# wzf2000/GAMER

Hardware: AMD Instinct MI355X
Metric: train-step sequences/sec, Qwen3Multi SMB decoder, his_len=100 (higher is better)
Workload: dtype f32 tensors/accumulators, products = 3 x fp16 pieces (split3)

## Files before the change

### gamer_amd/csrc/attention_common.h

```cpp
#pragma once
#include "common.h"
#include <stdlib.h>

namespace gamer {

constexpr int AT_THREADS = 256;
constexpr int KLD = 68;
constexpr int INT_BIG_A = 0x7fffffff;

typedef float f32x16 __attribute__((ext_vector_type(16)));
__device__ __forceinline__ int rowmap(int reg, int h) { return (reg & 3) + 8 * (reg >> 2) + 4 * h; }

struct RowOrder {
    const int32_t* perm;
    const int32_t* tile_kind;
    const int32_t* tile_maxpos;
    const int32_t* span;
};

struct QuerySpan {
    int hi, hole_lo, hole_hi;
    template <bool SPAN>
    static __device__ __forceinline__ QuerySpan load(const int32_t* __restrict__ span, int64_t tok, int pos, bool valid, int S) {
        QuerySpan q;
// ... 68 lines not shown
            v.x = ok ? v.x : 0.f; v.y = ok ? v.y : 0.f; v.z = ok ? v.z : 0.f; v.w = ok ? v.w : 0.f;
            *reinterpret_cast<float4*>(lds + (f >> 4) * LD + ((f & 15) << 2)) = v;
        }
    }
}

struct KeyMeta {
    int32_t kl[32];
    uint32_t kw[32];
    int32_t klmax;
    int32_t pad_[3];
};

template <bool DROP>
__device__ __forceinline__ int key_meta_load(const int32_t* __restrict__ klb, int j0, int S, int w, int lane,
                                             const AttnDropout& rng) {
    const int j = j0 + (lane & 31);
    int v = 0;
    if (w == 0 || w == 1) {
        v = j < S ? klb[j] : INT_BIG_A;
    } else if (w == 2) {
        if (DROP) v = (int)rng.key_word((uint32_t)j);
    }
    return v;
}
__device__ __forceinline__ void key_meta_store(KeyMeta& km, int w, int lane, int v) {
    if (w == 0) { if (lane < 32) km.kl[lane] = v; }
    else if (w == 1) { v = wave_max_i32(v); if (lane == 0) km.klmax = v; }
    else if (w == 2) { if (lane < 32) km.kw[lane] = (uint32_t)v; }
}

__device__ __forceinline__ void read_key_quads(const int32_t* __restrict__ base, int h, int (&out)[16]) {
#pragma unroll
    for (int g4 = 0; g4 < 4; ++g4) {
        const int4 t = *reinterpret_cast<const int4*>(base + 8 * g4 + 4 * h);
        out[4 * g4] = t.x; out[4 * g4 + 1] = t.y; out[4 * g4 + 2] = t.z; out[4 * g4 + 3] = t.w;
    }
}

constexpr float RESCALE_TAU = 20.f;

template <typename T>
struct AttnFwdArgs {
    const T* q; int ldq; const T* k; int ldk; const T* v; int ldv;
    const int32_t* kl; const int32_t* ql; const int32_t* row_empty;
    int B, S, nq, nkv; float scale, p_drop; uint64_t seed;
    T* o; float* lse;
    RowOrder ro; int uspan;
    hipStream_t st;
};
template <typename T>
struct AttnBwdArgs {
    const T* q; int ldq; const T* k; int ldk; const T* v; int ldv;
    const T* o; const T* d_o; const float* lse; float* delta;
    const int32_t* kl; const int32_t* ql; const int32_t* row_empty; const int32_t* tile_empty;
    int B, S, nq, nkv; float scale, p_drop; uint64_t seed;
    T* dq; int lddq; T* dk; int lddk; T* dv; int lddv;
    RowOrder ro; float* ds_work; int delta_ready;
    hipStream_t st;
};
template <typename F>
static inline int with_group(int nq, int nkv, F&& f) {
    return nq / nkv == 1 ? f(std::integral_constant<int, 1>{}) : f(std::integral_constant<int, 2>{});
}

static inline int check_attn(const char* name, bool bf16, const void* q, const void* k, const void* v, const void* kl,
                             const void* row_empty, int ldq, int ldk, int ldv, int B, int S, int nq, int nkv, float p_drop) {
    GAMER_CHECK_ARG(q && k && v && kl && (bf16 || row_empty), "%s: null pointer", name);
    GAMER_CHECK_ARG(B > 0 && S > 0 && nq > 0 && nkv > 0 && nq % nkv == 0, "%s: bad shape B=%d S=%d nq=%d nkv=%d", name, B, S, nq, nkv);
    const int G = nq / nkv, m = bf16 ? 8 : 4;
    GAMER_CHECK_ARG(G == 1 || G == 2, "%s: GQA group %d not built (1 or 2)", name, G);
    GAMER_CHECK_ARG(ldq % m == 0 && ldk % m == 0 && ldv % m == 0 && ldq >= nq * 64 && ldk >= nkv * 64 && ldv >= nkv * 64,
                    "%s: bad leading dims ldq=%d ldk=%d ldv=%d%s", name, ldq, ldk, ldv, bf16 ? " (multiples of 8)" : "");
    GAMER_CHECK_ARG(aligned16(q) && aligned16(k) && aligned16(v), "%s: q/k/v must be 16-byte aligned", name);
    GAMER_CHECK_ARG(p_drop >= 0.f && p_drop < 1.f, "%s: p_drop=%f", name, p_drop);
    return 0;
}

static inline bool res_enabled() {
    static EnvSwitch sw("GAMER_ATTN_RES");
    return sw.get(1) != 0;
}
#define GAMER_RES_PART(name) ([]() -> bool { static EnvSwitch sw(name); return sw.get(1) != 0; }())
static inline int res_grid_cap() {
    static EnvSwitch grid("GAMER_ATTN_RES_GRID");
    if (grid.get(0) > 0) return grid.get(0);
    static int cap[MAX_DEVICES] = {};
    int& c = cap[current_device()];
    if (c == 0) {
        int n = 0;
        if (hipDeviceGetAttribute(&n, hipDeviceAttributeMultiprocessorCount, current_device()) != hipSuccess) n = 256;
        c = n > 0 ? n : 256;
    }
    return c;
}
static inline int res_split(int n_pairs, int ways) {
    if (ways < 2) return 0;
    static EnvSwitch sp("GAMER_ATTN_RES_SPLIT");
    if (sp.is_set()) return sp.get(0) != 0;
    const int ncu = res_grid_cap();
    const double whole = (double)((n_pairs + ncu - 1) / ncu), halves = 0.58 * (double)((ways * n_pairs + ncu - 1) / ncu);
    return halves < whole ? 1 : 0;
}
static inline bool res_split_forced() { static EnvSwitch sp("GAMER_ATTN_RES_SPLIT"); return sp.is_set(); }
static inline double res_fill(int n_pairs) {
    const int ncu = res_grid_cap();
    if (n_pairs <= ncu) return 1.0;
    return (double)n_pairs / ((double)((n_pairs + ncu - 1) / ncu) * ncu);
}
static inline dim3 res_grid(int n_units) { return dim3(n_units < res_grid_cap() ? n_units : res_grid_cap()); }

}
```

### gamer_amd/csrc/attention_res.hip

```cpp
#include "attention_split_common.h"

namespace gamer {

#ifndef RES_WARM
#define RES_WARM 0
#endif
#ifndef RES_TOUCH_Q
#define RES_TOUCH_Q 0
#endif
#ifndef RES_PREFETCH_Q
#define RES_PREFETCH_Q 0
#endif
#ifndef RES_STAMP
#define RES_STAMP 0
#endif
#if RES_STAMP
__device__ unsigned long long* g_res_stamp = nullptr;
#define RES_MARK(i) do { __builtin_amdgcn_sched_barrier(0); const unsigned long long t_ = __builtin_amdgcn_s_memtime(); \
                         ph_[i] += (t_ - tprev_); tprev_ = t_; __builtin_amdgcn_sched_barrier(0); } while (0)
#define RES_STAMP_ARGS , unsigned long long (&ph_)[8], unsigned long long& tprev_
#define RES_STAMP_PASS , ph_, tprev_
#else
#define RES_MARK(i) do { } while (0)
#define RES_STAMP_ARGS
// ... 272 lines not shown
#pragma unroll
            for (int reg = 0; reg < 16; ++reg) {
                float pe = __builtin_amdgcn_exp2f(st[reg]);
                if (EMPTYSEL) pe = my_empty ? 1.f : pe;
                rowsum += pe;
                st[reg] = pe;
            }
            rowsum = xor32_sum(rowsum);
            l_run += rowsum;
            if (DROP) {
                int kwv[16];
                read_key_quads(kwt, h, kwv);
#pragma unroll
                for (int reg = 0; reg < 16; ++reg) st[reg] = rng.keep(aw, (uint32_t)kwv[reg]) ? st[reg] : 0.f;
            }
            pv_tile.template operator()<false>();
        };
        if (wave_all_empty) {
            int kwv[16];
            if (DROP) read_key_quads(kwt, h, kwv);
#pragma unroll
            for (int reg = 0; reg < 16; ++reg) {
                const bool on = DROP ? rng.keep(aw, (uint32_t)kwv[reg]) : true;
                st[reg] = on ? 1.f : 0.f;
            }
            pv_tile.template operator()<true>();
        } else if (wave_has_empty) {
            softmax_tile.template operator()<true, true>();
        } else {
            const int klmax = __builtin_amdgcn_readfirstlane(sm.klmax[tl]);
            const bool free_tile = (j0 + 31 <= wave_q_lo) && (klmax < wave_ql_min) &&
                                   (!SPAN || j0 + 31 < wave_hole_lo || j0 >= wave_hole_hi);
            if (free_tile) softmax_tile.template operator()<false, false>();
            else softmax_tile.template operator()<true, false>();
        }
#if RES_STAMP
        ph_[6] += 1;
#endif
    }
    RES_MARK(2);

    if (last) {
        float omax = 0.f;
        if (valid_q) {
            float linv = my_empty ? invS : (l_run > 0.f ? 1.f / l_run : 0.f);
            if (DROP) linv *= rng.scale;
            linv *= H2Scales::INV_P * sc.inv_v;
#pragma unroll
            for (int dh = 0; dh < 2; ++dh)
#pragma unroll
                for (int g4 = 0; g4 < 4; ++g4) {
                    float4 t4;
                    t4.x = oacc[dh][4 * g4 + 0] * linv; t4.y = oacc[dh][4 * g4 + 1] * linv;
                    t4.z = oacc[dh][4 * g4 + 2] * linv; t4.w = oacc[dh][4 * g4 + 3] * linv;
                    *reinterpret_cast<float4*>(orow + 32 * dh + 8 * g4 + 4 * h) = t4;
                    omax = fmaxf(fmaxf(fmaxf(omax, fabsf(t4.x)), fabsf(t4.y)), fmaxf(fabsf(t4.z), fabsf(t4.w)));
                }
            if (h == 0) *lse_p = my_empty ? 0.f : (m_ref + __log2f(l_run)) * 0.6931471805599453f;
        }
        if (want_amax) {
            uint32_t mw = __float_as_uint(omax);
#pragma unroll
            for (int o2 = 32; o2 > 0; o2 >>= 1) mw = max(mw, (uint32_t)__shfl_xor((int)mw, o2, 64));
            if (lane == 0 && mw) atomicMax(&sm.amax_word, mw);
        }
    } else if (valid_q) {
        float f = my_empty ? 1.f : (l_run > 0.f ? 1.f / l_run : 0.f);
        f *= H2Scales::INV_P * sc.inv_v;
#pragma unroll
        for (int dh = 0; dh < 2; ++dh)
#pragma unroll
            for (int g4 = 0; g4 < 4; ++g4) {
                float4 t4;
                t4.x = oacc[dh][4 * g4 + 0] * f; t4.y = oacc[dh][4 * g4 + 1] * f;
                t4.z = oacc[dh][4 * g4 + 2] * f; t4.w = oacc[dh][4 * g4 + 3] * f;
                *reinterpret_cast<float4*>(orow + 32 * dh + 8 * g4 + 4 * h) = t4;
            }
        if (h == 0) *lse_p = my_empty ? 0.f : m_ref + __log2f(l_run);
    }
    asm volatile("" :: "v"(tq), "v"(tm));
    RES_MARK(3);
}

template <int G, bool DROP, bool SPAN, bool ORD>
__global__ void __launch_bounds__(RES_THREADS, 1)
attn_fwd_r_kernel(const float* __restrict__ q, int ldq, const float* __restrict__ k, int ldk, const float* __restrict__ v, int ldv,
                  const int32_t* __restrict__ kl, const int32_t* __restrict__ ql, const int32_t* __restrict__ row_empty,
                  int nbatch, int S, int nq, int nkv, float scale, float p_drop, uint64_t seed, float* o, float* lse,
                  const RowOrder ro, uint32_t* __restrict__ amax_out, const AttnAmax am, const int split) {
    extern __shared__ __attribute__((aligned(16))) unsigned char res_raw[];
    ResSmem& sm = *reinterpret_cast<ResSmem*>(res_raw);
    const H2Scales sc(am.q, am.k, am.v, nullptr, scale * 1.4426950408889634f);
    const AttnDropout rng(p_drop, seed);
    const int tid = threadIdx.x;
    const int n_all = (S + 31) >> 5;
    const int nblk = (S + RB_KEYS - 1) / RB_KEYS;
    const int hpu = split ? 1 : G, upp = G / hpu;
    const int n_items = hpu * n_all;
    const int n_pairs = nbatch * nkv * upp;
    const int lane = tid & 63, r = lane & 31;
    if (tid == 0) sm.amax_word = 0;
#if RES_STAMP
    unsigned long long ph_[8] = {0, 0, 0, 0, 0, 0, 0, 0};
    unsigned long long tprev_ = __builtin_amdgcn_s_memtime();
#endif
#pragma unroll 1
    for (int pair = blockIdx.x; pair < n_pairs; pair += gridDim.x) {
        const int b = (pair / upp) / nkv, kvh = (pair / upp) % nkv, h0 = (pair % upp) * hpu;
        const float* kbase = k + (int64_t)b * S * ldk + kvh * 64;
        const float* vbase = v + (int64_t)b * S * ldv + kvh * 64;
        const int32_t* klb = kl + (int64_t)b * S;
#pragma unroll 1
        for (int kb = 0; kb < nblk; ++kb) {
            RES_MARK(5);
            __syncthreads();
            RES_MARK(4);
            if (tid == 0) sm.ctr = 0;
            res_stage_block<DROP>(sm, kbase, ldk, vbase, ldv, klb, kb * RB_KEYS, S, tid, sc, rng);
            __syncthreads();
            RES_MARK(0);
            uint32_t tk0 = 0, tk1 = 0;
            {
                int npair = pair, nkb = kb + 1;
                if (nkb == nblk) { nkb = 0; npair += gridDim.x; }
                if (RES_WARM && npair < n_pairs) {
                    const int j = min(nkb * RB_KEYS + (tid >> 1), S - 1);
                    const int64_t nrow = (int64_t)((npair / upp) / nkv) * S + j;
                    tk0 = *reinterpret_cast<const uint32_t*>(k + nrow * ldk + ((npair / upp) % nkv) * 64 + (tid & 1) * 32);
                    tk1 = *reinterpret_cast<const uint32_t*>(v + nrow * ldv + ((npair / upp) % nkv) * 64 + (tid & 1) * 32);
                }
            }
            int cur = res_grab(sm, lane);
            int perm_cur = 0;
            float4 qraw[8];
            bool q_ready = false;
            if (ORD && cur < n_items) perm_cur = ro.perm[(int64_t)b * S + min((n_all - 1 - cur / hpu) * 32 + r, S - 1)];
#pragma unroll 1
            while (cur < n_items) {
                const int nxt = res_grab(sm, lane);
                const int hg = h0 + cur % hpu, t = n_all - 1 - cur / hpu;
                ResNext nx;
                nx.t = n_all - 1 - nxt / hpu;
                nx.head = kvh * G + h0 + nxt % hpu;
                nx.valid = nxt < n_items && (kb == 0 || sm.ntot[(h0 + nxt % hpu) * RES_MAX_TILES + nx.t] > kb * RB_TILES);
                nx.perm = 0;
                if (ORD && nxt < n_items) nx.perm = ro.perm[(int64_t)b * S + min(nx.t * 32 + r, S - 1)];
                if (kb == 0 || sm.ntot[hg * RES_MAX_TILES + t] > kb * RB_TILES) {
                    res_fwd_rowtile<G, DROP, ORD, SPAN>(sm, q, ldq, ql, row_empty, S, nq, scale, rng, o, lse, ro, b, kvh * G + hg, t, kb,
                                                  amax_out != nullptr, sc, perm_cur, nx, qraw, q_ready RES_STAMP_PASS);
                    q_ready = RES_PREFETCH_Q && nx.valid;
                } else {
                    q_ready = false;
                }
                cur = nxt;
                perm_cur = nx.perm;
            }
            asm volatile("" :: "v"(tk0), "v"(tk1));
        }
    }
    if (amax_out) {
        __syncthreads();
        if (tid == 0 && sm.amax_word) amax_publish(sm.amax_word, amax_out, blockIdx.x);
    }
#if RES_STAMP
    RES_MARK(5);
    if (g_res_stamp && (tid & 63) == 0) {
        unsigned long long* rec = g_res_stamp + ((size_t)blockIdx.x * 8 + (tid >> 6)) * 8;
#pragma unroll
        for (int i_ = 0; i_ < 8; ++i_) rec[i_] += ph_[i_];
    }
#endif
}


template <int G, bool DROP, bool ORD, bool SPAN>
__device__ __forceinline__ void
res_dq_rowtile(ResSmem& sm, const float* __restrict__ q, int ldq, const float* __restrict__ o, const float* __restrict__ d_o,
               const float* __restrict__ lse, float* delta, const int32_t* __restrict__ ql, const int32_t* __restrict__ row_empty,
               int S, int nq, float scale, const AttnDropout& rng, float* dq, int lddq, const RowOrder& ro, const int b,
               const int head, const int t, const int kb, const int delta_ready, const H2Scales& sc) {
    const int lane = threadIdx.x & 63;
    const int r = lane & 31, h = lane >> 5;
    const SlOffsets lo(lane);
    const int n_all = (S + 31) >> 5;
    const int slot = t * 32 + r;
    const bool valid_q = slot < S;
    const int slotc = valid_q ? slot : S - 1;
    const int iqc = ORD ? ro.perm[(int64_t)b * S + slotc] : slotc;
    const int iq = valid_q ? iqc : S;
    const int64_t tok = (int64_t)b * S + iqc;

    const bool need_delta = !delta_ready && kb == 0;
    float* delta_p = delta + ((int64_t)b * nq + head) * S + iqc;
    float* dqrow = dq + tok * lddq + head * 64;
    float4 qraw[8], draw[8];
    {
        const float* qrow = q + tok * ldq + head * 64 + 8 * h;
        const float* drow = d_o + tok * (int64_t)nq * 64 + head * 64 + 8 * h;
#pragma unroll
        for (int s = 0; s < 4; ++s) {
            qraw[2 * s] = *reinterpret_cast<const float4*>(qrow + 16 * s);
            qraw[2 * s + 1] = *reinterpret_cast<const float4*>(qrow + 16 * s + 4);
            draw[2 * s] = *reinterpret_cast<const float4*>(drow + 16 * s);
            draw[2 * s + 1] = *reinterpret_cast<const float4*>(drow + 16 * s + 4);
        }
    }
    const int my_ql = ql ? ql[tok] : 1;
    const bool my_empty = valid_q && row_empty[tok] != 0;
    const float my_lse = lse[((int64_t)b * nq + head) * S + iqc];
    float my_delta = 0.f;
    if (!need_delta) my_delta = __builtin_nontemporal_load(delta_p);
    f32x4v carry[8];
    if (kb > 0) {
#pragma unroll
        for (int i = 0; i < 8; ++i) {
            carry[i] = f32x4v{0.f, 0.f, 0.f, 0.f};
            if (valid_q) carry[i] = __builtin_nontemporal_load(reinterpret_cast<const f32x4v*>(dqrow + 32 * (i >> 2) + 8 * (i & 3) + 4 * h));
        }
    }
    const bool normal = valid_q && !my_empty;
    const QuerySpan sp = QuerySpan::load<SPAN>(ro.span, tok, iq, valid_q, S);
    const int wave_ql_min = wave_min_i32_dpp(normal ? my_ql : INT_BIG_A);
    const int wave_q_lo = wave_min_i32_dpp(normal ? sp.hi : INT_BIG_A);
    const bool wave_all_empty = wave_q_lo == INT_BIG_A;
    const int wave_hole_lo = SPAN ? wave_min_i32_dpp(normal ? sp.hole_lo : INT_BIG_A) : INT_BIG_A;
    const int wave_hole_hi = SPAN ? wave_max_i32_dpp(normal ? sp.hole_hi : 0) : 0;
    int wave_q_hi;
    bool wave_has_empty;
    if (ORD) {
        wave_q_hi = ro.tile_maxpos[(int64_t)b * n_all + t];
        wave_has_empty = (ro.tile_kind[(int64_t)b * n_all + t] & 2) != 0;
    } else {
        wave_q_hi = wave_all_empty ? -1 : min(S - 1, t * 32 + 31);
        wave_has_empty = __any(my_empty ? 1 : 0) != 0;
    }
    const int n_total = wave_has_empty ? n_all : (wave_q_hi < 0 ? 0 : (wave_q_hi >> 5) + 1);
    const int jt_lo = kb * RB_TILES;
    if (kb > 0 && jt_lo >= n_total) return;
    const int jt_hi = min(n_total, jt_lo + RB_TILES);
    const bool first = kb == 0, last = jt_lo + RB_TILES >= n_total;
    if (first && lane == 0) sm.ntot[(head % G) * RES_MAX_TILES + t] = n_total;

    const float qs = scale * 1.4426950408889634f;
    bf16x8 qf[2][4], dof[2][4];
    float my_sdo = sc.d_o, my_inv_do = sc.inv_do, my_sds = sc.ds, my_inv_ds = sc.inv_ds;
    {
        const float* orow = o + tok * (int64_t)nq * 64 + head * 64 + 8 * h;
        float4 du[4], dw[4];
        float rowmax = 0.f;
#pragma unroll
        for (int s = 0; s < 4; ++s) {
            float4 a4 = qraw[2 * s];
            float4 b4 = qraw[2 * s + 1];
            a4.x *= qs; a4.y *= qs; a4.z *= qs; a4.w *= qs; b4.x *= qs; b4.y *= qs; b4.z *= qs; b4.w *= qs;
            bf16x8 pq[3];
            cut8_t<true>(a4, b4, sc.q, pq);
            qf[0][s] = pq[0]; qf[1][s] = pq[1];
            float4 u4 = draw[2 * s];
            float4 w4 = draw[2 * s + 1];
            if (need_delta) {
                const float4 o4 = *reinterpret_cast<const float4*>(orow + 16 * s);
                const float4 p4 = *reinterpret_cast<const float4*>(orow + 16 * s + 4);
                my_delta += u4.x * o4.x + u4.y * o4.y + u4.z * o4.z + u4.w * o4.w + w4.x * p4.x + w4.y * p4.y + w4.z * p4.z + w4.w * p4.w;
            }
            if (!valid_q) { u4 = make_float4(0.f, 0.f, 0.f, 0.f); w4 = u4; }
            du[s] = u4; dw[s] = w4;
            rowmax = fmaxf(fmaxf(fmaxf(rowmax, fabsf(u4.x)), fabsf(u4.y)), fmaxf(fabsf(u4.z), fabsf(u4.w)));
            rowmax = fmaxf(fmaxf(fmaxf(rowmax, fabsf(w4.x)), fabsf(w4.y)), fmaxf(fabsf(w4.z), fabsf(w4.w)));
        }
        rowmax = xor32_max(rowmax);
        if (rowmax > 0.f) {
            scale_from_amax(__float_as_uint(rowmax), my_sdo, my_inv_do);
            scale_from_amax(__float_as_uint(sc.ds_coef * rowmax), my_sds, my_inv_ds);
        }
#pragma unroll
        for (int s = 0; s < 4; ++s) {
            bf16x8 dpc[3];
            cut8_t<true>(du[s], dw[s], my_sdo, dpc);
            dof[0][s] = dpc[0]; dof[1][s] = dpc[1];
        }
        if (need_delta) {
            my_delta = xor32_sum(my_delta);
            if (valid_q && h == 0) *delta_p = my_delta;
        }
    }
    const float neg_lse2 = -my_lse * 1.4426950408889634f;
    const float invS = 1.f / (float)S;
    const uint32_t aw = DROP ? rng.row_word((uint32_t)(((int64_t)b * nq + head) * S + iqc)) : 0u;
    const float sd = rng.scale;
    const float neg_delta = -my_delta;

    f32x16 dqacc[2];
    if (first) {
#pragma unroll
        for (int i = 0; i < 16; ++i) { dqacc[0][i] = 0.f; dqacc[1][i] = 0.f; }
    } else {
#pragma unroll
        for (int dh = 0; dh < 2; ++dh)
#pragma unroll
            for (int g4 = 0; g4 < 4; ++g4) {
                const f32x4v t4 = carry[4 * dh + g4];
                dqacc[dh][4 * g4 + 0] = t4[0]; dqacc[dh][4 * g4 + 1] = t4[1]; dqacc[dh][4 * g4 + 2] = t4[2]; dqacc[dh][4 * g4 + 3] = t4[3];
            }
    }

#pragma unroll 1
    for (int jt = jt_lo; jt < jt_hi; ++jt) {
        const int j0 = jt * 32, tl = jt - jt_lo;
        const bool beyond = j0 > wave_q_hi;
        if (beyond && !wave_has_empty) continue;
        const bf16_t* k0 = sm.K[0] + tl * SIMG;
        const bf16_t* k1 = sm.K[1] + tl * SIMG;
        const bf16_t* v0 = sm.V[0] + tl * SIMG;
        const bf16_t* v1 = sm.V[1] + tl * SIMG;
        const int32_t* klt = sm.kl + tl * 32;
        const int32_t* kwt = reinterpret_cast<const int32_t*>(sm.kw) + tl * 32;
        f32x16 st, dp;
        const float st0 = !beyond ? neg_lse2 * (sc.q * sc.k) : neg_lse2;
#pragma unroll
        for (int i = 0; i < 16; ++i) { st[i] = st0; dp[i] = 0.f; }
        {
            bf16x8 vf[2][2];
            vf[0][0] = *reinterpret_cast<const bf16x8*>(v0 + lo.row[0]);
            vf[0][1] = *reinterpret_cast<const bf16x8*>(v1 + lo.row[0]);
#pragma unroll
            for (int s = 0; s < 4; ++s) {
                if (s + 1 < 4) {
                    vf[(s + 1) & 1][0] = *reinterpret_cast<const bf16x8*>(v0 + lo.row[s + 1]);
                    vf[(s + 1) & 1][1] = *reinterpret_cast<const bf16x8*>(v1 + lo.row[s + 1]);
                }
                __builtin_amdgcn_sched_barrier(0);
                dp = mfma_piece<true>(vf[s & 1][1], dof[0][s], dp);
                dp = mfma_piece<true>(vf[s & 1][0], dof[1][s], dp);
                dp = mfma_piece<true>(vf[s & 1][0], dof[0][s], dp);
                __builtin_amdgcn_sched_barrier(0);
            }
        }
        if (!beyond && !wave_all_empty) st = res_qk_tile(sm, tl, lo, qf, st);
        {
            const float cdp = sc.inv_v * my_inv_do;
#pragma unroll
            for (int i = 0; i < 16; ++i) dp[i] *= cdp;
            if (!beyond) {
#pragma unroll
                for (int i = 0; i < 16; ++i) st[i] *= sc.inv_qk;
            }
        }
        __builtin_amdgcn_sched_barrier(0);
        if (DROP) {
            int kwv[16];
            read_key_quads(kwt, h, kwv);
#pragma unroll
            for (int reg = 0; reg < 16; ++reg) {
                const float tt = rng.keep(aw, (uint32_t)kwv[reg]) ? dp[reg] : 0.f;
                dp[reg] = fmaf(tt, sd, neg_delta);
            }
        } else {
#pragma unroll
            for (int reg = 0; reg < 16; ++reg) dp[reg] += neg_delta;
        }
        auto ds_tile = [&]<bool MASK, bool EMPTYSEL>() {
            if (MASK) {
                int klv[16];
                read_key_quads(klt, h, klv);
                const int t_pos = sp.hi - j0 - 4 * h;
                const int t_lo = sp.hole_lo - j0 - 4 * h, t_hi = sp.hole_hi - j0 - 4 * h;
#pragma unroll
                for (int reg = 0; reg < 16; ++reg) {
                    const int ko = (reg & 3) + 8 * (reg >> 2);
                    bool allowed = (ko <= t_pos) & (klv[reg] < my_ql);
                    if (SPAN) allowed = allowed & !((ko >= t_lo) & (ko < t_hi));
                    st[reg] = allowed ? st[reg] : -INFINITY;
                }
            }
#pragma unroll
            for (int reg = 0; reg < 16; ++reg) {
                float pe = __builtin_amdgcn_exp2f(st[reg]);
                if (EMPTYSEL) pe = my_empty ? 1.f : pe;
                st[reg] = pe * dp[reg];
            }
        };
        if (wave_all_empty) {
            st = dp;
        } else if (wave_has_empty) {
            ds_tile.template operator()<true, true>();
        } else {
            const int klmax = __builtin_amdgcn_readfirstlane(sm.klmax[tl]);
            const bool free_tile = (j0 + 31 <= wave_q_lo) && (klmax < wave_ql_min) &&
                                   (!SPAN || j0 + 31 < wave_hole_lo || j0 >= wave_hole_hi);
            if (free_tile) ds_tile.template operator()<false, false>();
            else ds_tile.template operator()<true, false>();
        }
        __builtin_amdgcn_sched_barrier(0);
#pragma unroll
        for (int s2 = 0; s2 < 2; ++s2) {
            bf16x8 df[3];
            cut8_regs_t<true>(st, 8 * s2, my_sds, df);
#pragma unroll
            for (int db = 0; db < 2; ++db) {
                bf16x8 kf[3];
                kf[0] = read_tr8(k0, lo, 16 * s2, db);
                kf[1] = read_tr8(k1, lo, 16 * s2, db);
                kf[2] = kf[1];
                dqacc[db] = mfma_pieces<true>(kf, df, dqacc[db]);
            }
        }
    }

    if (valid_q) {
        float fs = 1.f;
        if (last) fs = (my_empty ? scale * invS : scale) * (my_inv_ds * sc.inv_k);
#pragma unroll
        for (int dh = 0; dh < 2; ++dh)
#pragma unroll
            for (int g4 = 0; g4 < 4; ++g4) {
                float4 t4;
                t4.x = dqacc[dh][4 * g4 + 0] * fs; t4.y = dqacc[dh][4 * g4 + 1] * fs;
                t4.z = dqacc[dh][4 * g4 + 2] * fs; t4.w = dqacc[dh][4 * g4 + 3] * fs;
                *reinterpret_cast<float4*>(dqrow + 32 * dh + 8 * g4 + 4 * h) = t4;
            }
    }
}

template <int G, bool DROP, bool SPAN, bool ORD>
__global__ void __launch_bounds__(RES_THREADS, 1)
attn_bwd_dq_r_kernel(const float* __restrict__ q, int ldq, const float* __restrict__ k, int ldk, const float* __restrict__ v, int ldv,
                     const float* __restrict__ o, const float* __restrict__ d_o, const float* __restrict__ lse, float* delta,
                     const int32_t* __restrict__ kl, const int32_t* __restrict__ ql, const int32_t* __restrict__ row_empty,
                     int nbatch, int S, int nq, int nkv, float scale, float p_drop, uint64_t seed, float* dq, int lddq,
                     const RowOrder ro, const int delta_ready, const AttnAmax am, const int split) {
    extern __shared__ __attribute__((aligned(16))) unsigned char res_raw[];
    ResSmem& sm = *reinterpret_cast<ResSmem*>(res_raw);
    const H2Scales sc(am.q, am.k, am.v, am.d_o, scale * 1.4426950408889634f, 1.f / (1.f - p_drop));
    const AttnDropout rng(p_drop, seed);
    const int tid = threadIdx.x, lane = tid & 63;
    const int n_all = (S + 31) >> 5;
    const int nblk = (S + RB_KEYS - 1) / RB_KEYS;
    const int hpu = split ? 1 : G, upp = G / hpu;
    const int n_items = hpu * n_all;
    const int n_units = nbatch * nkv * upp;
#pragma unroll 1
    for (int unit = blockIdx.x; unit < n_units; unit += gridDim.x) {
        const int b = (unit / upp) / nkv, kvh = (unit / upp) % nkv, h0 = (unit % upp) * hpu;
        const float* kbase = k + (int64_t)b * S * ldk + kvh * 64;
        const float* vbase = v + (int64_t)b * S * ldv + kvh * 64;
        const int32_t* klb = kl + (int64_t)b * S;
#pragma unroll 1
        for (int kb = 0; kb < nblk; ++kb) {
            __syncthreads();
            if (tid == 0) sm.ctr = 0;
            res_stage_block<DROP>(sm, kbase, ldk, vbase, ldv, klb, kb * RB_KEYS, S, tid, sc, rng);
            __syncthreads();
            uint32_t tk0 = 0, tk1 = 0;
            {
                int nunit = unit, nkb = kb + 1;
                if (nkb == nblk) { nkb = 0; nunit += gridDim.x; }
                if (RES_WARM && nunit < n_units) {
                    const int j = min(nkb * RB_KEYS + (tid >> 1), S - 1);
                    const int64_t nrow = (int64_t)((nunit / upp) / nkv) * S + j;
                    tk0 = *reinterpret_cast<const uint32_t*>(k + nrow * ldk + ((nunit / upp) % nkv) * 64 + (tid & 1) * 32);
                    tk1 = *reinterpret_cast<const uint32_t*>(v + nrow * ldv + ((nunit / upp) % nkv) * 64 + (tid & 1) * 32);
                }
            }
#pragma unroll 1
            for (int cur = res_grab(sm, lane); cur < n_items; cur = res_grab(sm, lane)) {
                const int hg = h0 + cur % hpu, t = n_all - 1 - cur / hpu;
                if (kb == 0 || sm.ntot[hg * RES_MAX_TILES + t] > kb * RB_TILES)
                    res_dq_rowtile<G, DROP, ORD, SPAN>(sm, q, ldq, o, d_o, lse, delta, ql, row_empty, S, nq, scale, rng, dq, lddq, ro, b,
                                                 kvh * G + hg, t, kb, delta_ready, sc);
            }
            asm volatile("" :: "v"(tk0), "v"(tk1));
        }
    }
}


struct DkvRSmem {
    bf16_t Q[2][RIMG];
    bf16_t dO[2][RIMG];
    float nlse2[RB_KEYS];
    float ndelta[RB_KEYS];
    uint32_t aw[RB_KEYS];
    int32_t ql[RB_KEYS];
    int32_t empty[RB_KEYS];
    int32_t pos[RB_KEYS];
    int32_t t_qlmin[RB_TILES];
    int32_t t_posmin[RB_TILES];
    int32_t t_maxpos[RB_TILES];
    int32_t t_empty[RB_TILES];
    int32_t started[RES_MAX_TILES];
    uint32_t amax_word;
    int32_t ctr;
    int32_t pad_[6];
};

constexpr int DKV_R_THREADS = 256;
template <bool DROP, bool ORD>
__device__ __forceinline__ void
res_stage_queries(DkvRSmem& sm, const float* __restrict__ q, int ldq, const float* __restrict__ d_o, const float* __restrict__ lse,
                  const float* delta, const int32_t* __restrict__ ql, const int32_t* __restrict__ row_empty, const RowOrder& ro,
                  int b, int head, int s0, int S, int nq, int tid, const H2Scales& sc, const AttnDropout& rng) {
    const int32_t* pmap = ORD ? ro.perm + (int64_t)b * S : nullptr;
    float4 rq[8], rd[8];
    auto load8 = [&](int p0) {
#pragma unroll
        for (int p = 0; p < 8; ++p) {
            const int f = tid + DKV_R_THREADS * (p0 + p);
            const int sl = min(s0 + (f >> 4), S - 1);
            const int64_t tok = (int64_t)b * S + (ORD ? pmap[sl] : sl);
            rq[p] = *reinterpret_cast<const float4*>(q + tok * ldq + head * 64 + ((f & 15) << 2));
            rd[p] = *reinterpret_cast<const float4*>(d_o + tok * (int64_t)nq * 64 + head * 64 + ((f & 15) << 2));
        }
    };
    auto store8 = [&](int p0) {
#pragma unroll
        for (int p = 0; p < 8; ++p) {
            const int f = tid + DKV_R_THREADS * (p0 + p);
            const int row = f >> 4;
            const bool ok = s0 + row < S;
            const int off = sl_off(row, (f & 15) << 2);
            uint32_t a0, a1, b0, b1;
            cut2h_quad(ok ? rq[p].x : 0.f, ok ? rq[p].y : 0.f, ok ? rq[p].z : 0.f, ok ? rq[p].w : 0.f, sc.q, a0, a1, b0, b1);
            *reinterpret_cast<uint2*>(sm.Q[0] + off) = make_uint2(a0, b0);
            *reinterpret_cast<uint2*>(sm.Q[1] + off) = make_uint2(a1, b1);
            cut2h_quad(ok ? rd[p].x : 0.f, ok ? rd[p].y : 0.f, ok ? rd[p].z : 0.f, ok ? rd[p].w : 0.f, sc.d_o, a0, a1, b0, b1);
            *reinterpret_cast<uint2*>(sm.dO[0] + off) = make_uint2(a0, b0);
            *reinterpret_cast<uint2*>(sm.dO[1] + off) = make_uint2(a1, b1);
        }
    };
    load8(0);
    if (tid < RB_KEYS) {
        const int sl = s0 + tid;
        const bool in = sl < S;
        const int pos = in ? (ORD ? pmap[sl] : sl) : 0;
        const int64_t hrow = ((int64_t)b * nq + head) * S + pos;
        const int em = in ? row_empty[(int64_t)b * S + pos] : 0;
        const int qlv = in ? (ql ? ql[(int64_t)b * S + pos] : 1) : 0;
        sm.nlse2[tid] = in ? -lse[hrow] * 1.4426950408889634f : 0.f;
        sm.ndelta[tid] = in ? -delta[hrow] : 0.f;
        if (DROP) sm.aw[tid] = rng.row_word((uint32_t)hrow);
        sm.ql[tid] = qlv;
        sm.empty[tid] = em;
        sm.pos[tid] = in ? pos : S;
        const bool normal = in && em == 0;
        int qlmin = normal ? qlv : INT_BIG_A, posmin = normal ? pos : INT_BIG_A, maxpos = normal ? pos : -1, anye = em != 0 ? 1 : 0;
#pragma unroll
        for (int o2 = 16; o2 > 0; o2 >>= 1) {
            qlmin = min(qlmin, __shfl_xor(qlmin, o2, 64));
            posmin = min(posmin, __shfl_xor(posmin, o2, 64));
            maxpos = max(maxpos, __shfl_xor(maxpos, o2, 64));
            anye |= __shfl_xor(anye, o2, 64);
        }
// ... 681 lines not shown
            uint32_t tw[4] = {0, 0, 0, 0};
            if (RES_WARM && !ORD) {
                int npair = pair, nqb_ = qb + 1;
                if (nqb_ == nqb) { nqb_ = 0; npair += gridDim.x; }
                if (npair < n_pairs) {
                    const int sl = min(nqb_ * QB2 + (tid >> 1), S - 1);
                    const int64_t ntok = (int64_t)((npair / upp) / nkv) * S + sl;
                    const int nh0 = ((npair / upp) % nkv) * 2;
#pragma unroll
                    for (int g = 0; g < 2; ++g) {
                        tw[2 * g] = *reinterpret_cast<const uint32_t*>(q + ntok * ldq + (nh0 + g) * 64 + (tid & 1) * 32);
                        tw[2 * g + 1] = *reinterpret_cast<const uint32_t*>(d_o + ntok * (int64_t)nq * 64 + (nh0 + g) * 64 + (tid & 1) * 32);
                    }
                }
            }
            const bool final_stage = qb == nqb - 1;
            const int n_qt = min(QB2_TILES, n_all - qb * QB2_TILES);
            int blk_maxpos = -1, blk_empty = 0;
#pragma unroll 1
            for (int i = 0; i < n_qt; ++i) { blk_maxpos = max(blk_maxpos, sm.t_maxpos[i]); blk_empty |= sm.t_empty[i]; }
            blk_maxpos = __builtin_amdgcn_readfirstlane(blk_maxpos);
            blk_empty = __builtin_amdgcn_readfirstlane(blk_empty);
            auto needed = [&](int kt_) { return final_stage || blk_empty != 0 || blk_maxpos >= kt_ * 32; };
            bool first = true;
#pragma unroll 1
            while (true) {
                int kt = -1;
                if (RES_KEEP && first && held >= 0 && needed(held)) {
                    kt = held;
                } else {
                    int c = upp * res_grab_ctr(&sm.ctr, lane) + kt0;
                    while (RES_KEEP && c < n_all && __builtin_amdgcn_readfirstlane(sm.keeper_stage[c]) >= qb) c = upp * res_grab_ctr(&sm.ctr, lane) + kt0;
                    if (c < n_all && needed(c)) kt = c;
                }
                first = false;
                const bool release = held >= 0 && kt != held && (kt >= 0 || final_stage);
                const bool acquire = kt >= 0 && kt != held;
                if (!release && kt < 0) break;
                const bool fresh = acquire && __builtin_amdgcn_readfirstlane(sm.started[kt]) == 0;
                RES_MARK(5);
                res2_dkv_step<DROP, SPAN>(sm, k, ldk, v, ldv, kl, S, scale, rng, dk, lddk, dv, lddv, b, kvh, held, release, final_stage, kt,
                                          acquire, fresh, n_qt, amax_out != nullptr, sc, T RES_STAMP_PASS);
                if (release) held = -1;
                if (kt < 0) break;
                if (acquire && lane == 0) sm.started[kt] = 1;
                held = kt;
                if (!RES_KEEP) {
                    res2_dkv_step<DROP, SPAN>(sm, k, ldk, v, ldv, kl, S, scale, rng, dk, lddk, dv, lddv, b, kvh, held, true, final_stage, -1,
                                              false, false, n_qt, amax_out != nullptr, sc, T RES_STAMP_PASS);
                    held = -1;
                }
            }
            if (RES_KEEP && held >= 0 && lane == 0) sm.keeper_stage[held] = qb + 1;
            asm volatile("" :: "v"(tw[0]), "v"(tw[1]), "v"(tw[2]), "v"(tw[3]));
        }
    }
    if (amax_out) {
        __syncthreads();
        if (tid == 0 && sm.amax_word) amax_publish(sm.amax_word, amax_out, blockIdx.x);
    }
#if RES_STAMP
    RES_MARK(5);
    if (g_res_stamp && lane == 0) {
        unsigned long long* rec = g_res_stamp + ((size_t)blockIdx.x * 8 + (tid >> 6)) * 8;
#pragma unroll
        for (int i_ = 0; i_ < 8; ++i_) rec[i_] += ph_[i_];
    }
#endif
}

template <typename F>
static int with_res_variant(int nq, int nkv, float p_drop, const RowOrder& ro, F&& f) {
    const bool drop = p_drop > 0.f, ord = ro.perm != nullptr;
    if (ro.span) return with_flags([&](auto d, auto o) { return f(std::integral_constant<int, 2>{}, d, std::true_type{}, o); }, drop, ord);
    return with_group(nq, nkv, [&](auto g) { return with_flags([&](auto d, auto o) { return f(g, d, std::false_type{}, o); }, drop, ord); });
}

int launch_fwd_res(const AttnFwdArgs<float>& a, uint32_t* amax_out, AttnAmax am) {
    return with_res_variant(a.nq, a.nkv, a.p_drop, a.ro, [&](auto g, auto drop, auto span, auto ord) {
        const int split = res_split(a.B * a.nkv, g());
        return launch<attn_fwd_r_kernel<g(), drop(), span(), ord()>>("gamer_attn_fwd_split/resident", res_grid(a.B * a.nkv * (split ? g() : 1)),
                                                                     dim3(RES_THREADS), sizeof(ResSmem), a.st, a.q, a.ldq, a.k, a.ldk, a.v, a.ldv, a.kl,
                                                                     a.ql, a.row_empty, a.B, a.S, a.nq, a.nkv, a.scale, a.p_drop, a.seed, a.o, a.lse,
                                                                     a.ro, amax_out, am, split);
    });
}

int launch_dq_res(const AttnBwdArgs<float>& a, AttnAmax am) {
    return with_res_variant(a.nq, a.nkv, a.p_drop, a.ro, [&](auto g, auto drop, auto span, auto ord) {
        const int split = res_split(a.B * a.nkv, g());
        return launch<attn_bwd_dq_r_kernel<g(), drop(), span(), ord()>>("gamer_attn_bwd_split/dq resident", res_grid(a.B * a.nkv * (split ? g() : 1)),
                                                                        dim3(RES_THREADS), sizeof(ResSmem), a.st, a.q, a.ldq, a.k, a.ldk, a.v, a.ldv,
                                                                        a.o, a.d_o, a.lse, a.delta, a.kl, a.ql, a.row_empty, a.B, a.S, a.nq, a.nkv,
                                                                        a.scale, a.p_drop, a.seed, a.dq, a.lddq, a.ro, a.delta_ready, am, split);
    });
}

int launch_dkv_res(const AttnBwdArgs<float>& a, uint32_t* amax_out, AttnAmax am) {
    return with_res_variant(a.nq, a.nkv, a.p_drop, a.ro, [&](auto g, auto drop, auto span, auto ord) {
        const int n_pairs = a.B * a.nkv;
        GAMER_TRY(ensure_dynamic_lds<attn_bwd_dkv_r_kernel<g(), drop(), ord()>>("gamer_attn_bwd_split/dkv resident", sizeof(DkvRSmem)));
        if (g() == 2 && (span() || GAMER_RES_PART("GAMER_ATTN_RES_DKV2"))) {
            const int split = res_split(n_pairs, 2);
            return launch<attn_bwd_dkv_r2_kernel<drop(), span(), ord()>>("gamer_attn_bwd_split/dkv resident, two heads per wave",
                                                                         res_grid(n_pairs * (split ? 2 : 1)), dim3(DKV_R_THREADS), sizeof(DkvR2Smem),
                                                                         a.st, a.q, a.ldq, a.k, a.ldk, a.v, a.ldv, a.d_o, a.lse, a.delta, a.kl, a.ql,
                                                                         a.row_empty, a.B, a.S, a.nq, a.nkv, a.scale, a.p_drop, a.seed, a.dk, a.lddk,
                                                                         a.dv, a.lddv, a.ro, amax_out, am, split);
        }
        if constexpr (!span())
            return launch<attn_bwd_dkv_r_kernel<g(), drop(), ord()>>("gamer_attn_bwd_split/dkv resident", res_grid(n_pairs), dim3(DKV_R_THREADS),
                                                                     sizeof(DkvRSmem), a.st, a.q, a.ldq, a.k, a.ldk, a.v, a.ldv, a.d_o, a.lse, a.delta,
                                                                     a.kl, a.ql, a.row_empty, a.B, a.S, a.nq, a.nkv, a.scale, a.p_drop, a.seed, a.dk,
                                                                     a.lddk, a.dv, a.lddv, a.ro, amax_out, am);
        return 0;
    });
}

}

#if RES_STAMP
extern "C" int gamer_debug_res_stamp(void* p) {
    unsigned long long* v = (unsigned long long*)p;
    return (int)hipMemcpyToSymbol(HIP_SYMBOL(gamer::g_res_stamp), &v, sizeof(v));
}
#endif
```

Measured before the change: 5098.

## Add fast path for fully-masked row tiles in resident attention fwd and dq

Result: no change. 5136, median of 6 (+0.7%).

```diff
diff --git a/gamer_amd/csrc/attention_common.h b/gamer_amd/csrc/attention_common.h
--- a/gamer_amd/csrc/attention_common.h
+++ b/gamer_amd/csrc/attention_common.h
@@ -174,6 +174,7 @@
     return sw.get(1) != 0;
 }
 #define GAMER_RES_PART(name) ([]() -> bool { static EnvSwitch sw(name); return sw.get(1) != 0; }())
+static inline bool res_empty2() { return GAMER_RES_PART("GAMER_ATTN_RES_EMPTY2"); }
 static inline int res_grid_cap() {
     static EnvSwitch grid("GAMER_ATTN_RES_GRID");
     if (grid.get(0) > 0) return grid.get(0);
diff --git a/gamer_amd/csrc/attention_res.hip b/gamer_amd/csrc/attention_res.hip
--- a/gamer_amd/csrc/attention_res.hip
+++ b/gamer_amd/csrc/attention_res.hip
@@ -378,12 +378,123 @@
     RES_MARK(3);
 }
 
+__device__ __forceinline__ int res_empty_tail(const RowOrder& ro, int b, int n_all, int lane) {
+    const int kind = lane < n_all ? ro.tile_kind[(int64_t)b * n_all + lane] : 0;
+    const unsigned long long other = ~__ballot(kind == 2) & (n_all >= 64 ? ~0ull : ((1ull << n_all) - 1ull));
+    return other ? n_all - 1 - (63 - __builtin_clzll(other)) : n_all;
+}
+__device__ __forceinline__ uint32_t res_keep_pair(bool k0, bool k1) { return (k0 ? 0x7000u : 0u) | (k1 ? 0x70000000u : 0u); }
+
+template <bool DROP>
+__device__ __forceinline__ void
+res_fwd_rowtile_empty2(ResSmem& sm, int S, int nq, const AttnDropout& rng, float* o, float* lse, const int b, const int head0,
+                       const int t, const int kb, const bool want_amax, const H2Scales& sc, const RowOrder& ro) {
+    const int lane = threadIdx.x & 63;
+    const int r = lane & 31, h = lane >> 5;
+    const SlOffsets lo(lane);
+    const int n_all = (S + 31) >> 5;
+    const bool valid_q = t * 32 + r < S;
+    const int perm_cur = ro.perm[(int64_t)b * S + min(t * 32 + r, S - 1)];
+    const int64_t tok = (int64_t)b * S + perm_cur;
+    const int jt_lo = kb * RB_TILES;
+    const int jt_hi = min(n_all, jt_lo + RB_TILES);
+    const bool first = kb == 0, last = jt_lo + RB_TILES >= n_all;
+    if (first && lane == 0) { sm.ntot[t] = n_all; sm.ntot[RES_MAX_TILES + t] = n_all; }
+    float* orow[2];
+    float* lse_p[2];
+    uint32_t aw[2];
+    f32x16 oacc[2][2];
+#pragma unroll
+    for (int g = 0; g < 2; ++g) {
+        const int head = head0 + g;
+        orow[g] = o + tok * (int64_t)nq * 64 + head * 64;
+        lse_p[g] = lse + ((int64_t)b * nq + head) * S + perm_cur;
+        aw[g] = DROP ? rng.row_word((uint32_t)(((int64_t)b * nq + head) * S + perm_cur)) : 0u;
+    }
+    if (first) {
+#pragma unroll
+        for (int g = 0; g < 2; ++g)
+#pragma unroll
+            for (int i = 0; i < 16; ++i) { oacc[g][0][i] = 0.f; oacc[g][1][i] = 0.f; }
+    } else {
+        const float up = H2Scales::P * sc.v;
+#pragma unroll
+        for (int g = 0; g < 2; ++g)
+#pragma unroll
+            for (int dh = 0; dh < 2; ++dh)
+#pragma unroll
+                for (int g4 = 0; g4 < 4; ++g4) {
+                    f32x4v t4 = f32x4v{0.f, 0.f, 0.f, 0.f};
+                    if (valid_q) t4 = __builtin_nontemporal_load(reinterpret_cast<const f32x4v*>(orow[g] + 32 * dh + 8 * g4 + 4 * h));
+                    oacc[g][dh][4 * g4 + 0] = t4[0] * up; oacc[g][dh][4 * g4 + 1] = t4[1] * up;
+                    oacc[g][dh][4 * g4 + 2] = t4[2] * up; oacc[g][dh][4 * g4 + 3] = t4[3] * up;
+                }
+    }
+#pragma unroll 1
+    for (int jt = jt_lo; jt < jt_hi; ++jt) {
+        const int tl = jt - jt_lo;
+        const bf16_t* v0 = sm.V[0] + tl * SIMG;
+        const bf16_t* v1 = sm.V[1] + tl * SIMG;
+        int kwv[16];
+        if (DROP) read_key_quads(reinterpret_cast<const int32_t*>(sm.kw) + tl * 32, h, kwv);
+#pragma unroll
+        for (int s2 = 0; s2 < 2; ++s2) {
+            bf16x8 pf[2];
+#pragma unroll
+            for (int g = 0; g < 2; ++g) {
+                u32x4s u;
+#pragma unroll
+                for (int d = 0; d < 4; ++d) {
+                    const int reg = 8 * s2 + 2 * d;
+                    u[d] = DROP ? res_keep_pair(rng.keep(aw[g], (uint32_t)kwv[reg]), rng.keep(aw[g], (uint32_t)kwv[reg + 1])) : 0x70007000u;
+                }
+                pf[g] = __builtin_bit_cast(bf16x8, u);
+            }
+#pragma unroll
+            for (int db = 0; db < 2; ++db) {
+                const bf16x8 vf0 = read_tr8(v0, lo, 16 * s2, db);
+                const bf16x8 vf1 = read_tr8(v1, lo, 16 * s2, db);
+                oacc[0][db] = mfma_piece<true>(vf1, pf[0], oacc[0][db]);
+                oacc[1][db] = mfma_piece<true>(vf1, pf[1], oacc[1][db]);
+                oacc[0][db] = mfma_piece<true>(vf0, pf[0], oacc[0][db]);
+                oacc[1][db] = mfma_piece<true>(vf0, pf[1], oacc[1][db]);
+            }
+        }
+    }
+    float f = last ? 1.f / (float)S : 1.f;
+    if (last && DROP) f *= rng.scale;
+    f *= H2Scales::INV_P * sc.inv_v;
+    float omax = 0.f;
+    if (valid_q) {
+#pragma unroll
+        for (int g = 0; g < 2; ++g) {
+#pragma unroll
+            for (int dh = 0; dh < 2; ++dh)
+#pragma unroll
+                for (int g4 = 0; g4 < 4; ++g4) {
+                    float4 t4;
+                    t4.x = oacc[g][dh][4 * g4 + 0] * f; t4.y = oacc[g][dh][4 * g4 + 1] * f;
+                    t4.z = oacc[g][dh][4 * g4 + 2] * f; t4.w = oacc[g][dh][4 * g4 + 3] * f;
+                    *reinterpret_cast<float4*>(orow[g] + 32 * dh + 8 * g4 + 4 * h) = t4;
+                    omax = fmaxf(fmaxf(fmaxf(omax, fabsf(t4.x)), fabsf(t4.y)), fmaxf(fabsf(t4.z), fabsf(t4.w)));
+                }
+            if (h == 0) *lse_p[g] = 0.f;
+        }
+    }
+    if (last && want_amax) {
+        uint32_t mw = __float_as_uint(omax);
+#pragma unroll
+        for (int o2 = 32; o2 > 0; o2 >>= 1) mw = max(mw, (uint32_t)__shfl_xor((int)mw, o2, 64));
+        if (lane == 0 && mw) atomicMax(&sm.amax_word, mw);
+    }
+}
+
 template <int G, bool DROP, bool SPAN, bool ORD>
 __global__ void __launch_bounds__(RES_THREADS, 1)
 attn_fwd_r_kernel(const float* __restrict__ q, int ldq, const float* __restrict__ k, int ldk, const float* __restrict__ v, int ldv,
                   const int32_t* __restrict__ kl, const int32_t* __restrict__ ql, const int32_t* __restrict__ row_empty,
                   int nbatch, int S, int nq, int nkv, float scale, float p_drop, uint64_t seed, float* o, float* lse,
-                  const RowOrder ro, uint32_t* __restrict__ amax_out, const AttnAmax am, const int split) {
+                  const RowOrder ro, uint32_t* __restrict__ amax_out, const AttnAmax am, const int split, const int empty2) {
     extern __shared__ __attribute__((aligned(16))) unsigned char res_raw[];
     ResSmem& sm = *reinterpret_cast<ResSmem*>(res_raw);
     const H2Scales sc(am.q, am.k, am.v, nullptr, scale * 1.4426950408889634f);
@@ -392,9 +503,10 @@
     const int n_all = (S + 31) >> 5;
     const int nblk = (S + RB_KEYS - 1) / RB_KEYS;
     const int hpu = split ? 1 : G, upp = G / hpu;
-    const int n_items = hpu * n_all;
     const int n_pairs = nbatch * nkv * upp;
     const int lane = tid & 63, r = lane & 31;
+    constexpr bool CAN_PAIR = G == 2 && ORD && !SPAN;
+    const bool pair2 = CAN_PAIR && empty2 && !split;
     if (tid == 0) sm.amax_word = 0;
 #if RES_STAMP
     unsigned long long ph_[8] = {0, 0, 0, 0, 0, 0, 0, 0};
@@ -406,6 +518,9 @@
         const float* kbase = k + (int64_t)b * S * ldk + kvh * 64;
         const float* vbase = v + (int64_t)b * S * ldv + kvh * 64;
         const int32_t* klb = kl + (int64_t)b * S;
+        int n_e = 0;
+        if constexpr (CAN_PAIR) { if (pair2) n_e = res_empty_tail(ro, b, n_all, lane); }
+        const int n_rest = n_all - n_e, n_items = n_e + hpu * n_rest;
 #pragma unroll 1
         for (int kb = 0; kb < nblk; ++kb) {
             RES_MARK(5);
@@ -427,20 +542,27 @@
                 }
             }
             int cur = res_grab(sm, lane);
+            if constexpr (CAN_PAIR) {
+#pragma unroll 1
+                for (; cur < n_e; cur = res_grab(sm, lane))
+                    res_fwd_rowtile_empty2<DROP>(sm, S, nq, rng, o, lse, b, kvh * G, n_all - 1 - cur, kb, amax_out != nullptr, sc, ro);
+            }
+            cur -= n_e;
+            const int n_left = n_items - n_e;
             int perm_cur = 0;
             float4 qraw[8];
             bool q_ready = false;
-            if (ORD && cur < n_items) perm_cur = ro.perm[(int64_t)b * S + min((n_all - 1 - cur / hpu) * 32 + r, S - 1)];
-#pragma unroll 1
-            while (cur < n_items) {
-                const int nxt = res_grab(sm, lane);
-                const int hg = h0 + cur % hpu, t = n_all - 1 - cur / hpu;
+            if (ORD && cur < n_left) perm_cur = ro.perm[(int64_t)b * S + min((n_rest - 1 - cur / hpu) * 32 + r, S - 1)];
+#pragma unroll 1
+            while (cur < n_left) {
+                const int nxt = res_grab(sm, lane) - n_e;
+                const int hg = h0 + cur % hpu, t = n_rest - 1 - cur / hpu;
                 ResNext nx;
-                nx.t = n_all - 1 - nxt / hpu;
+                nx.t = n_rest - 1 - nxt / hpu;
                 nx.head = kvh * G + h0 + nxt % hpu;
-                nx.valid = nxt < n_items && (kb == 0 || sm.ntot[(h0 + nxt % hpu) * RES_MAX_TILES + nx.t] > kb * RB_TILES);
+                nx.valid = nxt < n_left && (kb == 0 || sm.ntot[(h0 + nxt % hpu) * RES_MAX_TILES + nx.t] > kb * RB_TILES);
                 nx.perm = 0;
-                if (ORD && nxt < n_items) nx.perm = ro.perm[(int64_t)b * S + min(nx.t * 32 + r, S - 1)];
+                if (ORD && nxt < n_left) nx.perm = ro.perm[(int64_t)b * S + min(nx.t * 32 + r, S - 1)];
                 if (kb == 0 || sm.ntot[hg * RES_MAX_TILES + t] > kb * RB_TILES) {
                     res_fwd_rowtile<G, DROP, ORD, SPAN>(sm, q, ldq, ql, row_empty, S, nq, scale, rng, o, lse, ro, b, kvh * G + hg, t, kb,
                                                   amax_out != nullptr, sc, perm_cur, nx, qraw, q_ready RES_STAMP_PASS);
@@ -474,7 +596,7 @@
 res_dq_rowtile(ResSmem& sm, const float* __restrict__ q, int ldq, const float* __restrict__ o, const float* __restrict__ d_o,
                const float* __restrict__ lse, float* delta, const int32_t* __restrict__ ql, const int32_t* __restrict__ row_empty,
                int S, int nq, float scale, const AttnDropout& rng, float* dq, int lddq, const RowOrder& ro, const int b,
-               const int head, const int t, const int kb, const int delta_ready, const H2Scales& sc) {
+               const int head, const int t, const int kb, const int delta_ready, const H2Scales& sc, const bool skip_empty) {
     const int lane = threadIdx.x & 63;
     const int r = lane & 31, h = lane >> 5;
     const SlOffsets lo(lane);
@@ -486,6 +608,9 @@
     const int iq = valid_q ? iqc : S;
     const int64_t tok = (int64_t)b * S + iqc;
 
+    int tkind = 0, tmaxpos = 0;
+    if (ORD) { tkind = ro.tile_kind[(int64_t)b * n_all + t]; tmaxpos = ro.tile_maxpos[(int64_t)b * n_all + t]; }
+    const bool tile_empty = ORD && !SPAN && skip_empty && tkind == 2;
     const bool need_delta = !delta_ready && kb == 0;
     float* delta_p = delta + ((int64_t)b * nq + head) * S + iqc;
     float* dqrow = dq + tok * lddq + head * 64;
@@ -495,15 +620,22 @@
         const float* drow = d_o + tok * (int64_t)nq * 64 + head * 64 + 8 * h;
 #pragma unroll
         for (int s = 0; s < 4; ++s) {
-            qraw[2 * s] = *reinterpret_cast<const float4*>(qrow + 16 * s);
-            qraw[2 * s + 1] = *reinterpret_cast<const float4*>(qrow + 16 * s + 4);
+            if (!tile_empty) {
+                qraw[2 * s] = *reinterpret_cast<const float4*>(qrow + 16 * s);
+                qraw[2 * s + 1] = *reinterpret_cast<const float4*>(qrow + 16 * s + 4);
+            }
             draw[2 * s] = *reinterpret_cast<const float4*>(drow + 16 * s);
             draw[2 * s + 1] = *reinterpret_cast<const float4*>(drow + 16 * s + 4);
         }
     }
-    const int my_ql = ql ? ql[tok] : 1;
-    const bool my_empty = valid_q && row_empty[tok] != 0;
-    const float my_lse = lse[((int64_t)b * nq + head) * S + iqc];
+    int my_ql = 1;
+    bool my_empty = valid_q;
+    float my_lse = 0.f;
+    if (!tile_empty) {
+        if (ql) my_ql = ql[tok];
+        my_empty = valid_q && row_empty[tok] != 0;
+        my_lse = lse[((int64_t)b * nq + head) * S + iqc];
+    }
     float my_delta = 0.f;
     if (!need_delta) my_delta = __builtin_nontemporal_load(delta_p);
     f32x4v carry[8];
@@ -524,8 +656,8 @@
     int wave_q_hi;
     bool wave_has_empty;
     if (ORD) {
-        wave_q_hi = ro.tile_maxpos[(int64_t)b * n_all + t];
-        wave_has_empty = (ro.tile_kind[(int64_t)b * n_all + t] & 2) != 0;
+        wave_q_hi = tmaxpos;
+        wave_has_empty = (tkind & 2) != 0;
     } else {
         wave_q_hi = wave_all_empty ? -1 : min(S - 1, t * 32 + 31);
         wave_has_empty = __any(my_empty ? 1 : 0) != 0;
@@ -546,12 +678,14 @@
         float rowmax = 0.f;
 #pragma unroll
         for (int s = 0; s < 4; ++s) {
-            float4 a4 = qraw[2 * s];
-            float4 b4 = qraw[2 * s + 1];
-            a4.x *= qs; a4.y *= qs; a4.z *= qs; a4.w *= qs; b4.x *= qs; b4.y *= qs; b4.z *= qs; b4.w *= qs;
-            bf16x8 pq[3];
-            cut8_t<true>(a4, b4, sc.q, pq);
-            qf[0][s] = pq[0]; qf[1][s] = pq[1];
+            if (!tile_empty) {
+                float4 a4 = qraw[2 * s];
+                float4 b4 = qraw[2 * s + 1];
+                a4.x *= qs; a4.y *= qs; a4.z *= qs; a4.w *= qs; b4.x *= qs; b4.y *= qs; b4.z *= qs; b4.w *= qs;
+                bf16x8 pq[3];
+                cut8_t<true>(a4, b4, sc.q, pq);
+                qf[0][s] = pq[0]; qf[1][s] = pq[1];
+            }
             float4 u4 = draw[2 * s];
             float4 w4 = draw[2 * s + 1];
             if (need_delta) {
@@ -614,7 +748,11 @@
         f32x16 st, dp;
         const float st0 = !beyond ? neg_lse2 * (sc.q * sc.k) : neg_lse2;
 #pragma unroll
-        for (int i = 0; i < 16; ++i) { st[i] = st0; dp[i] = 0.f; }
+        for (int i = 0; i < 16; ++i) dp[i] = 0.f;
+        if (!tile_empty) {
+#pragma unroll
+            for (int i = 0; i < 16; ++i) st[i] = st0;
+        }
         {
             bf16x8 vf[2][2];
             vf[0][0] = *reinterpret_cast<const bf16x8*>(v0 + lo.row[0]);
@@ -724,7 +862,7 @@
                      const float* __restrict__ o, const float* __restrict__ d_o, const float* __restrict__ lse, float* delta,
                      const int32_t* __restrict__ kl, const int32_t* __restrict__ ql, const int32_t* __restrict__ row_empty,
                      int nbatch, int S, int nq, int nkv, float scale, float p_drop, uint64_t seed, float* dq, int lddq,
-                     const RowOrder ro, const int delta_ready, const AttnAmax am, const int split) {
+                     const RowOrder ro, const int delta_ready, const AttnAmax am, const int split, const int empty2) {
     extern __shared__ __attribute__((aligned(16))) unsigned char res_raw[];
     ResSmem& sm = *reinterpret_cast<ResSmem*>(res_raw);
     const H2Scales sc(am.q, am.k, am.v, am.d_o, scale * 1.4426950408889634f, 1.f / (1.f - p_drop));
@@ -763,7 +901,7 @@
                 const int hg = h0 + cur % hpu, t = n_all - 1 - cur / hpu;
                 if (kb == 0 || sm.ntot[hg * RES_MAX_TILES + t] > kb * RB_TILES)
                     res_dq_rowtile<G, DROP, ORD, SPAN>(sm, q, ldq, o, d_o, lse, delta, ql, row_empty, S, nq, scale, rng, dq, lddq, ro, b,
-                                                 kvh * G + hg, t, kb, delta_ready, sc);
+                                                 kvh * G + hg, t, kb, delta_ready, sc, empty2 != 0);
             }
             asm volatile("" :: "v"(tk0), "v"(tk1));
         }
@@ -1611,7 +1749,7 @@
         return launch<attn_fwd_r_kernel<g(), drop(), span(), ord()>>("gamer_attn_fwd_split/resident", res_grid(a.B * a.nkv * (split ? g() : 1)),
                                                                      dim3(RES_THREADS), sizeof(ResSmem), a.st, a.q, a.ldq, a.k, a.ldk, a.v, a.ldv, a.kl,
                                                                      a.ql, a.row_empty, a.B, a.S, a.nq, a.nkv, a.scale, a.p_drop, a.seed, a.o, a.lse,
-                                                                     a.ro, amax_out, am, split);
+                                                                     a.ro, amax_out, am, split, (int)res_empty2());
     });
 }
 
@@ -1621,7 +1759,8 @@
         return launch<attn_bwd_dq_r_kernel<g(), drop(), span(), ord()>>("gamer_attn_bwd_split/dq resident", res_grid(a.B * a.nkv * (split ? g() : 1)),
                                                                         dim3(RES_THREADS), sizeof(ResSmem), a.st, a.q, a.ldq, a.k, a.ldk, a.v, a.ldv,
                                                                         a.o, a.d_o, a.lse, a.delta, a.kl, a.ql, a.row_empty, a.B, a.S, a.nq, a.nkv,
-                                                                        a.scale, a.p_drop, a.seed, a.dq, a.lddq, a.ro, a.delta_ready, am, split);
+                                                                        a.scale, a.p_drop, a.seed, a.dq, a.lddq, a.ro, a.delta_ready, am, split,
+                                                                        (int)res_empty2());
     });
 }
 
```
